# ocrickard/piper-swift

Hardware: AMD Instinct MI355X
Metric: audio-sec/wall-sec (RTF^-1) with ms/utterance, Piper VITS en_GB-medium geometry, scale-bench factor (higher is better)
Workload: dtype f32; 1 GPU; medium factor=8: 112 ids, 336 frames, 86016 samples (3.901 s audio) per utterance, 1 utterance per step per GPU; factor=8, phoneme_count=112, frames=336, samples=86016, parallelism=utterance-replicas x1 (one-shot RCCL weight broadcast)

## Files before the change

include/piper_hip.h:

```cpp
#ifndef PIPER_HIP_H
#define PIPER_HIP_H

#include <stddef.h>
#include <stdint.h>

#ifdef __cplusplus
extern "C" {
#endif

#define PIPER_HIP_ABI_VERSION 3

enum {
  PIPER_HIP_OK = 0,
  PIPER_HIP_ERR_SHAPE = -1,
  PIPER_HIP_ERR_TYPE = -2,
  PIPER_HIP_ERR_UNSUPPORTED = -3,
  PIPER_HIP_ERR_UNAVAILABLE = -4,
  PIPER_HIP_ERR_ALLOC = -5,
  PIPER_HIP_ERR_LAUNCH = -6,
  PIPER_HIP_ERR_ARG = -7
};

typedef struct piper_hip_ctx piper_hip_ctx;
typedef struct piper_hip_voice piper_hip_voice;
// ... 89 lines not shown
                               const int64_t* pads, float value, float** out, int64_t* out_shape,
                               piper_hip_stream stream);
int piper_hip_slice_f32(piper_hip_ctx* ctx, const float* x, const int64_t* shape, int rank, int axis, int64_t start,
                        int64_t end, int64_t step, float** out, int64_t* out_shape, piper_hip_stream stream);
int piper_hip_transpose_f32(piper_hip_ctx* ctx, const float* x, const int64_t* shape, int rank, const int32_t* perm,
                            float** out, int64_t* out_shape, piper_hip_stream stream);
int piper_hip_concat2_axis1_f32(piper_hip_ctx* ctx, const float* a, const int64_t a_shape[3], const float* b,
                                const int64_t b_shape[3], float** out, int64_t out_shape[3],
                                piper_hip_stream stream);
int piper_hip_split2_axis1_f32(piper_hip_ctx* ctx, const float* x, const int64_t x_shape[3], int64_t c0,
                               float** out0, float** out1, piper_hip_stream stream);
int piper_hip_expand_f32(piper_hip_ctx* ctx, const float* x, const int64_t* in_shape, const int64_t* out_shape,
                         int rank, float** out, piper_hip_stream stream);
int piper_hip_reduce_mean_lastdim_f32(piper_hip_ctx* ctx, const float* x, const int64_t* shape, int rank,
                                      float** out, piper_hip_stream stream);

int piper_hip_random_normal_like_f32(piper_hip_ctx* ctx, size_t count, uint64_t seed, float** out, piper_hip_stream stream);
int piper_hip_random_draws_u32(piper_hip_ctx* ctx, size_t count, uint64_t seed, uint32_t** out, piper_hip_stream stream);


int piper_hip_rel_attention_f32(piper_hip_ctx* ctx, const float* q, const float* k, const float* v,
                                const float* emb_rel_k, const float* emb_rel_v, int64_t n, int64_t heads,
                                int64_t head_dim, int64_t t, int64_t window, float** out, piper_hip_stream stream);

int piper_hip_attention_block_f32(piper_hip_ctx* ctx, const float* q, const float* k, const float* v, const float* emb_rel_k,
                                  const float* emb_rel_v, const float* w_o, const float* b_o, const float* x, const float* gamma,
                                  const float* beta, int64_t n, int64_t heads, int64_t head_dim, int64_t t, int64_t window, float eps,
                                  float** out, piper_hip_stream stream);

int piper_hip_add_layernorm_f32(piper_hip_ctx* ctx, const float* x, const float* y, const float* gamma,
                                const float* beta, int64_t n, int64_t c, int64_t t, float eps, float** out,
                                piper_hip_stream stream);

int piper_hip_wavenet_layer_f32(piper_hip_ctx* ctx, const float* x, const float* skip_in, const float* w_in,
                                const float* b_in, const float* w_rs, const float* b_rs, int64_t n, int64_t c,
                                int64_t t, int64_t k, int64_t dilation, int last, float** x_out, float** skip_out,
                                piper_hip_stream stream);

int piper_hip_hifigan_resblock_f32(piper_hip_ctx* ctx, int type, const float* x, int64_t n, int64_t c, int64_t t,
                                   int64_t k, const int32_t* dilations, int n_dil, const float* const* weights,
                                   const float* const* biases, float lrelu_slope, float** out,
                                   piper_hip_stream stream);


#define PIPER_HIP_MAX_UPS 4
#define PIPER_HIP_MAX_RB 3
// ... 266 lines not shown
```

piper-swift_amd/csrc/attention.hip:

```cpp
#include <algorithm>
#include <cstdlib>

#include "common.h"
#include "conv.h"

namespace {

constexpr int kBlock = 256;
constexpr int kKeyTile = 128;

__device__ __forceinline__ float wave_sum(float v) {
#pragma unroll
  for (int o = 32; o > 0; o >>= 1) v += __shfl_xor(v, o, 64);
  return v;
}
__device__ __forceinline__ float wave_max(float v) {
#pragma unroll
  for (int o = 32; o > 0; o >>= 1) v = fmaxf(v, __shfl_xor(v, o, 64));
  return v;
}

template <int R>
__global__ __launch_bounds__(kBlock) void rel_attention_kernel(const float* __restrict__ q, const float* __restrict__ k,
                                                               const float* __restrict__ v, const float* __restrict__ ek,
// ... 471 lines not shown
                    int T, int w, int64_t in_bs, int64_t out_bs, const int* len_ptr) {
  const int Tp = ((T + 31) / 32) * 32 + 2;
  const size_t lds = ((size_t)RV * Tp + 16 * 17) * sizeof(float);
  if (lds > 160 * 1024) return -1;
  static bool raised[ph::kMaxDevices] = {};
  if (lds > 64 * 1024 && ph::lds_optin_needed(raised))
    (void)hipFuncSetAttribute((const void*)rel_attention_mfma_kernel<D, RV>, hipFuncAttributeMaxDynamicSharedMemorySize, 160 * 1024);
  dim3 grid((unsigned)ph::ceil_div(T, RV), (unsigned)H, (unsigned)N);
  hipLaunchKernelGGL((rel_attention_mfma_kernel<D, RV>), grid, dim3(64 * kAttWaves), lds, s, q, k, v, ek, ev, out, T, w, in_bs, out_bs, len_ptr, Tp);
  return 0;
}

constexpr int kTK = 128;
constexpr int kLdK = kTK + 16;
constexpr int kLdV = kTK + 2;

#ifdef PH_ATT_LDS_TRACE
__device__ unsigned long long* ph_att_trace_buf;
#define PH_ASTAMP(k) do { if ((threadIdx.x & 63) == 0 && ph_att_trace_buf) ph_att_trace_buf[((size_t)(blockIdx.x + gridDim.x * blockIdx.y) * kAttWaves + (threadIdx.x >> 6)) * 8 + (k)] = __builtin_amdgcn_s_memtime(); } while (0)
#else
#define PH_ASTAMP(k) do { } while (0)
#endif
template <int D, bool SPLIT>
__global__ __launch_bounds__(64 * kAttWaves) void rel_attention_lds_kernel(const float* __restrict__ q, const float* __restrict__ k,
                                                                          const float* __restrict__ v, const float* __restrict__ ek,
                                                                          const float* __restrict__ ev, float* __restrict__ out, int T,
                                                                          int w, int64_t in_batch_stride, int64_t out_batch_stride,
                                                                          const int* __restrict__ len_ptr, int Tp, int nsplit,
                                                                          float* __restrict__ part_o, float* __restrict__ part_ml) {
  constexpr int RV = 16, NS = D / 4, NCT = D / 16;
  constexpr int NT = 64 * kAttWaves;
  constexpr int F4 = D * (kTK / 4);
  constexpr int SLOTS = (F4 + NT - 1) / NT;
  extern __shared__ __attribute__((aligned(16))) float smem[];
  float* tile = smem;
  float* sc = tile + D * kLdK;
  float* qs = sc + RV * Tp;
  float* qe = qs + D * 16;
  const int tid = threadIdx.x, lane = tid & 63;
  const int wave = __builtin_amdgcn_readfirstlane(tid >> 6);
  const int r16 = lane & 15, kq = lane >> 4;
  const int i0 = blockIdx.x * RV, n = blockIdx.z;
  const int h = SPLIT ? (int)blockIdx.y / nsplit : (int)blockIdx.y;
  const int part = SPLIT ? (int)blockIdx.y - h * nsplit : 0;
  const int Tv = len_ptr ? min(len_ptr[n], T) : T;
  if (i0 >= Tv) return;
  const int W = 2 * w + 1;
  const int64_t hoff = (int64_t)n * in_batch_stride + (int64_t)h * D * T;
  const float* qb = q + hoff;
  const float* kb = k + hoff;
  const float* vb = v + hoff;
  const float scale = sqrtf((float)D);
  const int ntile_all = (Tv + kTK - 1) / kTK;
  const int tpp = SPLIT ? (ntile_all + nsplit - 1) / nsplit : ntile_all;
  const int tb = SPLIT ? part * tpp : 0;
  const int te = SPLIT ? min(tb + tpp, ntile_all) : ntile_all;
  if (SPLIT && tb >= te) return;
  const int kbeg = tb * kTK, kend = min(te * kTK, Tv);
  const int ntile = te - tb;

  float4 stg[SLOTS];
  auto fetch = [&](const float* src, int t0) {
#pragma unroll
    for (int i = 0; i < SLOTS; i++) {
      const int e = tid + NT * i;
      const int row = min(e >> 5, D - 1), c4 = e & 31;
      const int col = min(t0 + 4 * c4, T - 4);
      stg[i] = *(const float4*)(src + (int64_t)row * T + col);
    }
  };
  auto commit = [&](int ld, int t0) {
#pragma unroll
    for (int i = 0; i < SLOTS; i++) {
      const int e = tid + NT * i;
      const int row = e >> 5, c4 = e & 31;
      if (row < D) {
        float4 val = stg[i];
        if (t0 + 4 * c4 > T - 4) val = make_float4(0.0f, 0.0f, 0.0f, 0.0f);
        float2* dst = (float2*)(tile + row * ld + 4 * c4);
        dst[0] = make_float2(val.x, val.y);
        dst[1] = make_float2(val.z, val.w);
      }
    }
  };

  PH_ASTAMP(0);
  fetch(kb, kbeg);
  for (int e = tid; e < D * 16; e += NT) {
    const int c = e >> 4, i = e & 15;
    const bool ok = i0 + i < Tv;
    const float qv = qb[(int64_t)c * T + min(i0 + i, Tv - 1)];
    qs[c * 16 + i] = ok ? qv / scale : 0.0f;
  }
  float arel[4];
  if (wave < NCT) {
#pragma unroll
    for (int s = 0; s < 4; s++) arel[s] = ev[min(4 * s + kq, W - 1) * D + wave * 16 + r16];
  }
  float ekf[NS];
  if (wave == kAttWaves - 1) {
    const int mc = min(r16, W - 1);
#pragma unroll
    for (int s = 0; s < NS; s++) ekf[s] = ek[mc * D + 4 * s + kq];
  }
  commit(kLdK, kbeg);
  PH_ASTAMP(1);
  __syncthreads();
  PH_ASTAMP(2);
  if (wave == kAttWaves - 1) {
    f32x4 a0 = {0.0f, 0.0f, 0.0f, 0.0f}, a1 = {0.0f, 0.0f, 0.0f, 0.0f};
#pragma unroll
    for (int s = 0; s < NS; s += 2) {
      a0 = __builtin_amdgcn_mfma_f32_16x16x4f32(qs[(4 * s + kq) * 16 + r16], r16 < W ? ekf[s] : 0.0f, a0, 0, 0, 0);
      a1 = __builtin_amdgcn_mfma_f32_16x16x4f32(qs[(4 * (s + 1) + kq) * 16 + r16], r16 < W ? ekf[s + 1] : 0.0f, a1, 0, 0, 0);
    }
#pragma unroll
    for (int r = 0; r < 4; r++) qe[(4 * kq + r) * 17 + r16] = a0[r] + a1[r];
  }

  for (int t = 0; t < ntile; t++) {
    const int t0 = kbeg + t * kTK;
    if (t + 1 < ntile) fetch(kb, t0 + kTK);
    else fetch(vb, kbeg);
    const int j0 = t0 + wave * 16;
    if (j0 < Tv) {
      const bool col_ok = j0 + r16 < Tv;
      f32x4 a0 = {0.0f, 0.0f, 0.0f, 0.0f}, a1 = {0.0f, 0.0f, 0.0f, 0.0f};
#pragma unroll
// ... 57 lines not shown
      row[j] = e;
      sum += e;
    }
    sum = wave_sum(sum);
    if constexpr (SPLIT) {
      if (lane == 0) {
        float* ml = part_ml + (((int64_t)n * gridDim.y + blockIdx.y) * 2) * T;
        ml[ia] = m;
        ml[T + ia] = sum;
      }
    } else {
      const float inv = 1.0f / sum;
      for (int j = lane; j < Tv; j += 64) row[j] *= inv;
    }
  }
  PH_ASTAMP(4);
  commit(kLdV, kbeg);
  __syncthreads();
  PH_ASTAMP(5);

  const bool pi_ok = i0 + r16 < Tv;
  const float* prow = sc + r16 * Tp;
  f32x4 acc = {0.0f, 0.0f, 0.0f, 0.0f}, accb = {0.0f, 0.0f, 0.0f, 0.0f};
  for (int t = 0; t < ntile; t++) {
    const int t0 = kbeg + t * kTK;
    if (t + 1 < ntile) fetch(vb, t0 + kTK);
    if (wave < NCT) {
      const float* vrow = tile + (wave * 16 + r16) * kLdV;
      const int nst = min(kTK, Tv - t0 + 3) >> 2;
      for (int s = 0; s < nst; s += 2) {
        const int j = t0 + 4 * s + kq;
        const bool ok = j < Tv, ok2 = j + 4 < Tv && s + 1 < nst;
        const float a0v = vrow[4 * s + kq], a1v = vrow[min(4 * (s + 1) + kq, kTK - 1)];
        const float b0v = prow[min(j, Tv - 1)], b1v = prow[min(j + 4, Tv - 1)];
        acc = __builtin_amdgcn_mfma_f32_16x16x4f32(ok ? a0v : 0.0f, (ok && pi_ok) ? b0v : 0.0f, acc, 0, 0, 0);
        accb = __builtin_amdgcn_mfma_f32_16x16x4f32(ok2 ? a1v : 0.0f, (ok2 && pi_ok) ? b1v : 0.0f, accb, 0, 0, 0);
      }
    }
    if (t + 1 < ntile) {
      __syncthreads();
      commit(kLdV, t0 + kTK);
      __syncthreads();
    }
  }
  if (wave < NCT) {
    const int ia = i0 + r16;
// ... 201 lines not shown
  const int Tp = ((T + 31) / 32) * 32 + 2;
  return ((size_t)2 * 16 * Tp + 2 * 16 * 17 + (size_t)H * d * 16 + kAttWaves * 16) * sizeof(float) <= 160 * 1024;
}

int launch_attention_block(piper_hip_ctx* ctx, hipStream_t s, const float* q, const float* k, const float* v, const float* ek, const float* ev,
                           const float* wo16, const float* bo, const float* xres, const float* gamma, const float* beta, float* out, int N,
                           int H, int d, int T, int w, int64_t in_batch_stride, int64_t x_batch_stride, const int* len_ptr, int o_nsteps,
                           float eps) {
  if (N <= 0 || T <= 0) return PIPER_HIP_OK;
  if (!attention_block_eligible(H, d, w, T) || N > 65535) PH_FAIL(PIPER_HIP_ERR_UNSUPPORTED, "attention_block: geometry not covered");
  if (launch_att_block<96>(s, q, k, v, ek, ev, wo16, bo, xres, gamma, beta, out, N, H, T, w, in_batch_stride, x_batch_stride, len_ptr, o_nsteps,
                           eps) != 0)
    PH_FAIL(PIPER_HIP_ERR_UNSUPPORTED, "attention_block: needs more than 160 KiB of LDS");
  PH_ROUTE(ctx, H * d, d, T, N, "att_block D=%d", d);
  hipError_t e = hipGetLastError();
  if (e != hipSuccess) PH_FAIL(PIPER_HIP_ERR_LAUNCH, "attention_block launch failed: %s", hipGetErrorString(e));
  return PIPER_HIP_OK;
}
}

PH_EXPORT int piper_hip_rel_attention_f32(piper_hip_ctx* ctx, const float* q, const float* k, const float* v,
                                          const float* emb_rel_k, const float* emb_rel_v, int64_t n, int64_t heads,
                                          int64_t head_dim, int64_t t, int64_t window, float** out, piper_hip_stream stream) {
  PH_CHECK_CTX(ctx);
  if (n < 0 || heads <= 0 || head_dim <= 0 || t < 0 || window < 0) PH_FAIL(PIPER_HIP_ERR_SHAPE, "rel_attention: bad shape");
  if (n * heads * head_dim * t > 0x7fffffff) PH_FAIL(PIPER_HIP_ERR_SHAPE, "rel_attention: tensor too large");
  const size_t cnt = (size_t)(n * heads * head_dim * t);
  int rc = ph::ensure_out(ctx, out, cnt, 0);
  if (rc) return rc;
  if (cnt == 0) return PIPER_HIP_OK;
  if (!q || !k || !v || !emb_rel_k || !emb_rel_v) PH_FAIL(PIPER_HIP_ERR_ARG, "rel_attention: null input");
  ph::StreamScope ss(ctx, stream);
  ph::RouteScope routes(ctx);
  const int64_t bs = heads * head_dim * t;
  const int nsplit = ph::rel_attention_split_parts(ctx, (int)n, (int)heads, (int)head_dim, (int)t, (int)window);
  if (nsplit > 1) {
    void *po = nullptr, *pml = nullptr;
    rc = ctx->pool.alloc((size_t)(n * heads * nsplit * head_dim * t) * sizeof(float), &po);
    if (rc) return rc;
    ph::defer_free(ctx, po);
    rc = ctx->pool.alloc((size_t)(n * heads * nsplit * 2 * t) * sizeof(float), &pml);
    if (rc) return rc;
    ph::defer_free(ctx, pml);
    rc = ph::launch_rel_attention_split(ctx, ss.s, q, k, v, emb_rel_k, emb_rel_v, *out, (int)n, (int)heads, (int)head_dim, (int)t, (int)window, bs,
                                        bs, nullptr, nsplit, (float*)po, (float*)pml);
  } else
    rc = ph::launch_rel_attention(ctx, ss.s, q, k, v, emb_rel_k, emb_rel_v, *out, (int)n, (int)heads, (int)head_dim, (int)t,
                                  (int)window, bs, bs, nullptr);
  if (rc) return rc;
  return ss.finish("rel_attention_f32");
}

PH_EXPORT int piper_hip_attention_block_f32(piper_hip_ctx* ctx, const float* q, const float* k, const float* v, const float* emb_rel_k,
                                            const float* emb_rel_v, const float* w_o, const float* b_o, const float* x,
                                            const float* gamma, const float* beta, int64_t n, int64_t heads, int64_t head_dim, int64_t t,
                                            int64_t window, float eps, float** out, piper_hip_stream stream) {
  PH_CHECK_CTX(ctx);
  if (n < 0 || heads <= 0 || head_dim <= 0 || t < 0 || window < 0) PH_FAIL(PIPER_HIP_ERR_SHAPE, "attention_block: bad shape");
  if (n * heads * head_dim * t > 0x7fffffff) PH_FAIL(PIPER_HIP_ERR_SHAPE, "attention_block: tensor too large");
  const int C = (int)(heads * head_dim);
  const size_t cnt = (size_t)(n * C * t);
  int rc = ph::ensure_out(ctx, out, cnt, 0);
  if (rc) return rc;
  if (cnt == 0) return PIPER_HIP_OK;
  if (!q || !k || !v || !emb_rel_k || !emb_rel_v || !w_o || !b_o || !x || !gamma || !beta) PH_FAIL(PIPER_HIP_ERR_ARG, "attention_block: null input");
  if (!ph::attention_block_eligible((int)heads, (int)head_dim, (int)window, (int)t))
    PH_FAIL(PIPER_HIP_ERR_UNSUPPORTED, "attention_block: covered geometry is head_dim 96, heads·head_dim ≤ 256, window ≤ 7, T ≤ 2048 — compose "
                                       "rel_attention + conv1d + add_layernorm instead");
  ph::StreamScope ss(ctx, stream);
  ph::RouteScope routes(ctx);
  void* pw = nullptr;
// ... 16 lines not shown
```

piper-swift_amd/csrc/prosody.hip:

```cpp
#include <algorithm>
#include <climits>
#include <cmath>

#include "common.h"
#include "dp_scalars.h"
#include "rng.h"

namespace ph {
namespace {

__global__ __launch_bounds__(256) void dp_final_prosody_kernel(const float* __restrict__ z, const float* __restrict__ m, const float* __restrict__ logs,
                                                               const DpScalars* __restrict__ sc, const float* __restrict__ len,
                                                               const int32_t* __restrict__ minf, const int32_t* __restrict__ maxf,
                                                               float* __restrict__ logw, float* __restrict__ w0_out, int32_t* __restrict__ dur, int T,
                                                               const int* __restrict__ len_ptr) {
  const int n = blockIdx.y;
  const int t = blockIdx.x * 256 + threadIdx.x;
  if (t >= T) return;
  const int64_t i = (int64_t)n * T + t;
  const float zv = z[(int64_t)n * 2 * T + t];
  const float lm = len[i];
  const int32_t mn = minf[i], mx = maxf[i];
  const float m0 = m[0], lg0 = logs[0], ls = sc[n].length_scale;
  const int Tv = len_ptr ? min(len_ptr[n], T) : T;
  float lw = 0.0f, w0 = 0.0f;
  int32_t d = 0;
  if (t < Tv) {
    lw = (zv - m0) * expf(-lg0);
// ... 74 lines not shown
    int32_t* tail = rep + n + (size_t)n * T;
    tail[b] = fitted ? 1 : 0;
    tail[n + 2 * b] = (int32_t)(unsigned)(S & 0xffffffffLL);
    tail[n + 2 * b + 1] = (int32_t)(S >> 32);
  }
  for (int f = tid; f < F; f += 256) {
    int id = 0;
    if (f < Fv && (long long)f < total) {
      int lo = 0, hi = Tb - 1;
      while (lo < hi) {
        const int mid = (lo + hi) >> 1;
        if (cum[mid] > f) hi = mid; else lo = mid + 1;
      }
      id = lo;
    }
    frame2id[(size_t)b * F + f] = id;
  }
}

__global__ __launch_bounds__(256) void expand_noise_prosody_kernel(const float* __restrict__ stats, const int32_t* __restrict__ frame2id,
                                                                   const float* __restrict__ noise, const float* __restrict__ id_noise,
                                                                   float* __restrict__ zp, float* __restrict__ zp_tap, int I, int T, int F,
                                                                   const float* __restrict__ noise_scale_dev, const unsigned* __restrict__ rng_dev,
                                                                   const int* __restrict__ lensF) {
  const int nb = blockIdx.y;
  stats += (int64_t)nb * 2 * I * T;
  frame2id += (int64_t)nb * F;
  noise += (int64_t)nb * I * F;
  id_noise += (int64_t)nb * T;
  zp += (int64_t)nb * I * F;
  zp_tap += (int64_t)nb * I * F;
  const float noise_scale = noise_scale_dev[nb];
  const bool gen = rng_dev[2 * nb] != 0u;
  const unsigned seed = rng_dev[2 * nb + 1];
  const int Fv = lensF ? min(lensF[nb], F) : F;
  const int64_t total = (int64_t)I * F;
  for (int64_t i = (int64_t)blockIdx.x * 256 + threadIdx.x; i < total; i += (int64_t)gridDim.x * 256) {
    const int c = (int)(i / F), f = (int)(i - (int64_t)c * F);
    const int t = frame2id[f];
    const float m = stats[(int64_t)c * T + t];
    const float lg = stats[(int64_t)(I + c) * T + t];
    const float pn = id_noise[t];
    const float nin = gen ? 0.0f : noise[i];
    const float nz = gen ? (f < Fv ? rnl_normal(seed, (unsigned)(c * Fv + f)) : 0.0f) : nin;
    const float ns = noise_scale * pn;
    const float r = m + (nz * expf(lg)) * ns;
    zp[i] = r;
    zp_tap[i] = r;
  }
}

const char* check_fields(const piper_hip_prosody* p, char* msg, size_t cap) {
  if (p->t < 1) { snprintf(msg, cap, "t = %d (at least 1)", p->t); return msg; }
  for (int i = 0; i < p->t; i++) {
    if (p->length && !(std::isfinite(p->length[i]) && p->length[i] >= 0.0f && p->length[i] <= 1000.0f)) {
      snprintf(msg, cap, "length[%d] = %g outside [0, 1000]", i, (double)p->length[i]);
      return msg;
    }
    if (p->noise && !(std::isfinite(p->noise[i]) && p->noise[i] >= 0.0f && p->noise[i] <= 1000.0f)) {
      snprintf(msg, cap, "noise[%d] = %g outside [0, 1000]", i, (double)p->noise[i]);
      return msg;
    }
    if (p->min_frames && (p->min_frames[i] < 0 || p->min_frames[i] > 1000000)) {
      snprintf(msg, cap, "min_frames[%d] = %d outside [0, 1000000]", i, p->min_frames[i]);
      return msg;
    }
    if (p->max_frames && (p->max_frames[i] < 0 || p->max_frames[i] > 1000000)) {
      snprintf(msg, cap, "max_frames[%d] = %d outside [0, 1000000]", i, p->max_frames[i]);
      return msg;
    }
    if (p->max_frames && p->min_frames && p->max_frames[i] != 0 && p->min_frames[i] > p->max_frames[i]) {
      snprintf(msg, cap, "min_frames[%d] = %d above max_frames[%d] = %d", i, p->min_frames[i], i, p->max_frames[i]);
// ... 13 lines not shown
    PH_FAIL(PIPER_HIP_ERR_ARG, "prosody: %s", why);
  }
  return PIPER_HIP_OK;
}

int launch_dp_final_prosody(hipStream_t s, const float* z, const float* m, const float* logs, const void* scalars, const float* len, const int32_t* minf,
                            const int32_t* maxf, float* logw, float* w0, int32_t* dur, int N, int T, const int* len_ptr) {
  const dim3 grid((unsigned)ceil_div(T, 256), (unsigned)N);
  hipLaunchKernelGGL(dp_final_prosody_kernel, grid, dim3(256), 0, s, z, m, logs, (const DpScalars*)scalars, len, minf, maxf, logw, w0, dur, T, len_ptr);
  return PIPER_HIP_OK;
}

size_t prosody_report_entries(int n, int T) { return (size_t)n + (size_t)n * T + 3 * (size_t)n; }

int launch_dp_paths_prosody(hipStream_t s, const int32_t* dur, const int* lensT, const int32_t* fit, int T, int F, int cap, int32_t* frame2id, int* lensF,
                            int32_t* rep, int n) {
  if (T > 4096 || !rep) PH_FAIL(PIPER_HIP_ERR_LAUNCH, "dp_paths_prosody: %d ids per row (at most 4096) or no report area", T);
  hipLaunchKernelGGL(dp_paths_prosody_kernel, dim3(n), dim3(256), 0, s, dur, lensT, fit, T, F, cap, frame2id, lensF, rep, n);
  return PIPER_HIP_OK;
}

int launch_expand_noise_prosody(hipStream_t s, const float* stats, const int32_t* frame2id, const float* noise, const float* id_noise, float* zp,
                                float* zp_tap, int NB, int I, int T, int F, const float* noise_scale, const unsigned* rng, const int* lensF) {
  const int grid = (int)std::min<int64_t>(ceil_div((int64_t)I * F, 256), 4096);
  hipLaunchKernelGGL(expand_noise_prosody_kernel, dim3(grid, NB), dim3(256), 0, s, stats, frame2id, noise, id_noise, zp, zp_tap, I, T, F, noise_scale, rng,
                     lensF);
  return PIPER_HIP_OK;
}

}
namespace ph { namespace { PH_WARM(prosody, dp_final_prosody_kernel); } }

using namespace ph;

PH_EXPORT int piper_hip_prosody_check(const piper_hip_prosody* p) { return prosody_check_item(p, -1); }

PH_EXPORT int piper_hip_prosody_frames(const piper_hip_prosody* p, const float* w0, int32_t t, int64_t cap, int32_t* frames_out, int64_t* wanted) {
  if (!w0 || !frames_out) PH_FAIL(PIPER_HIP_ERR_ARG, "prosody_frames: null argument");
  if (t < 1) PH_FAIL(PIPER_HIP_ERR_ARG, "prosody_frames: t = %d (at least 1)", t);
  if (p) {
    if (int rc = prosody_check_item(p, -1)) return rc;
    if (p->t != t) PH_FAIL(PIPER_HIP_ERR_SHAPE, "prosody_frames: the prosody has %d entries, the utterance %d ids", p->t, t);
  }
  int64_t S = 0;
  for (int i = 0; i < t; i++) {
    const float w1 = w0[i] * ((p && p->length) ? p->length[i] : 1.0f);
    const float c = ceilf(w1);
    const int32_t d0 = c > 0.0f ? (c < 1e6f ? (int32_t)c : 1000000) : 0;
    const int32_t mx = (p && p->max_frames) ? p->max_frames[i] : 0, mn = (p && p->min_frames) ? p->min_frames[i] : 0;
// ... 10 lines not shown
```

piper-swift_amd/csrc/voice.hip:

```cpp
#include <algorithm>
#include <cmath>
#include <cstdlib>
#include <chrono>
#include <functional>
#include <memory>

#include "../../include/piper_hip_voice_layout.h"
#include "conv.h"
#include "conv_bf16.h"
#include "conv_win.h"
#include "pcm16.h"
#include "resample.h"
#include "rng.h"
#include "speaker.h"

namespace ph {
int validate_config(const piper_hip_voice_config* c);
int validate_speaker_config(const piper_hip_voice_config* cfg, const piper_hip_speaker_config* sc);
int launch_rel_attention(piper_hip_ctx* ctx, hipStream_t s, const float* q, const float* k, const float* v, const float* ek,
                         const float* ev, float* out, int N, int H, int d, int T, int w, int64_t in_batch_stride,
                         int64_t out_batch_stride, const int* len_ptr);
int rel_attention_split_parts(piper_hip_ctx* ctx, int N, int H, int d, int T, int w);
int launch_rel_attention_split(piper_hip_ctx* ctx, hipStream_t s, const float* q, const float* k, const float* v, const float* ek,
                               const float* ev, float* out, int N, int H, int d, int T, int w, int64_t in_batch_stride,
                               int64_t out_batch_stride, const int* len_ptr, int nsplit, float* part_o, float* part_ml);
size_t dp_scalars_bytes(int n);
void dp_scalars_fill(void* host, int i, float noise_w, float length_scale, unsigned gen, unsigned seed);
bool flow_seam_eligible(int H, int half);
int launch_flow_seam(piper_hip_ctx* ctx, hipStream_t s, const float* skip, float* zp, float* h, const float* post16, const float* post_b, const float* pre16,
                     const float* pre_b, int N, int H, int half, int F, int post_steps, int pre_steps, int ob, int os, const int* len_ptr);
bool dds_layer_eligible(int H, int K);
int launch_dds_layer(piper_hip_ctx* ctx, hipStream_t s, const float* x, const float* dw_w, const float* dw_b, const float* g1, const float* b1,
                     const float* pw16, const float* pw_b, const float* g2, const float* b2, float* out, int N, int H, int T, int K, int dil,
// ... 21 lines not shown
using namespace ph;

namespace {

constexpr int kBlock = 256;
constexpr int kMaxSlots = 16;

__global__ __launch_bounds__(kBlock) void embed_kernel(const int64_t* __restrict__ ids, const float* __restrict__ emb,
                                                       float* __restrict__ x, int H, int T, int n_vocab, float scale) {
  ids += (int64_t)blockIdx.y * T;
  x += (int64_t)blockIdx.y * H * T;
  const int total = H * T;
  for (int i = blockIdx.x * kBlock + threadIdx.x; i < total; i += gridDim.x * kBlock) {
    const int c = i / T, t = i - c * T;
    int64_t id = ids[t];
    if (id < 0) id += n_vocab;
    x[i] = (id < 0 || id >= n_vocab) ? 0.0f * scale : emb[id * H + c] * scale;
  }
}

__global__ __launch_bounds__(kBlock) void expand_noise_kernel(const float* __restrict__ stats, const int32_t* __restrict__ frame2id,
                                                              const float* __restrict__ noise, float* __restrict__ zp, float* __restrict__ zp_tap,
                                                              int I, int T, int F, const float* __restrict__ noise_scale_dev,
                                                              const unsigned* __restrict__ rng_dev, const int* __restrict__ lensF) {
  const int nb = blockIdx.y;
  stats += (int64_t)nb * 2 * I * T;
  frame2id += (int64_t)nb * F;
  noise += (int64_t)nb * I * F;
  zp += (int64_t)nb * I * F;
  zp_tap += (int64_t)nb * I * F;
  const float noise_scale = noise_scale_dev[nb];
  const bool gen = rng_dev[2 * nb] != 0u;
  const unsigned seed = rng_dev[2 * nb + 1];
  const int Fv = lensF ? min(lensF[nb], F) : F;
  const int64_t total = (int64_t)I * F;
  for (int64_t i = (int64_t)blockIdx.x * kBlock + threadIdx.x; i < total; i += (int64_t)gridDim.x * kBlock) {
    const int c = (int)(i / F), f = (int)(i - (int64_t)c * F);
    const int t = frame2id[f];
    const float m = stats[(int64_t)c * T + t];
    const float lg = stats[(int64_t)(I + c) * T + t];
    const float nz = gen ? (f < Fv ? rnl_normal(seed, (unsigned)(c * Fv + f)) : 0.0f) : noise[i];
    const float r = m + (nz * expf(lg)) * noise_scale;
    zp[i] = r;
    zp_tap[i] = r;
  }
}

__global__ __launch_bounds__(kBlock) void mrf_mean_lrelu_kernel(const float* __restrict__ a, const float* __restrict__ b,
                                                                const float* __restrict__ c, float* __restrict__ y, int64_t n,
                                                                float alpha) {
  const int64_t n4 = n >> 2;
  const int64_t stride = (int64_t)gridDim.x * kBlock;
  for (int64_t i = (int64_t)blockIdx.x * kBlock + threadIdx.x; i < n4; i += stride) {
    const float4 va = reinterpret_cast<const float4*>(a)[i], vb = reinterpret_cast<const float4*>(b)[i],
                 vc = reinterpret_cast<const float4*>(c)[i];
    float4 r;
    r.x = ((va.x + vb.x) + vc.x) / 3.0f; r.y = ((va.y + vb.y) + vc.y) / 3.0f;
    r.z = ((va.z + vb.z) + vc.z) / 3.0f; r.w = ((va.w + vb.w) + vc.w) / 3.0f;
    r.x = r.x >= 0.0f ? r.x : alpha * r.x; r.y = r.y >= 0.0f ? r.y : alpha * r.y;
    r.z = r.z >= 0.0f ? r.z : alpha * r.z; r.w = r.w >= 0.0f ? r.w : alpha * r.w;
    reinterpret_cast<float4*>(y)[i] = r;
  }
  for (int64_t i = (n4 << 2) + (int64_t)blockIdx.x * kBlock + threadIdx.x; i < n; i += stride) {
    const float v = ((a[i] + b[i]) + c[i]) / 3.0f;
    y[i] = v >= 0.0f ? v : alpha * v;
  }
}

// ... 1381 lines not shown
    b.conv("enc.proj", v->proj, b.plain(x, stats, H, 2 * I, T, lensT), T);
  return PIPER_HIP_OK;
}

const float* build_flow(Builder& b, const FrontBuffers& fb) {
  piper_hip_voice* v = b.v;
  Slot& s = b.s;
  const int T = b.T, F = b.F, NB = b.NB;
  const int* lensF = b.lensF;
  const piper_hip_voice_config& c = v->cfg;
  const int H = c.hidden, I = c.inter;
  float *stats = fb.stats, *zp = fb.zp, *zflip = fb.zflip, *zp_tap = fb.zp_tap, *h = fb.h, *acts = fb.acts, *skip = fb.skip;
  {
    const int32_t* f2i = s.frame2id;
    const float* nz = s.noise;
    const float* nsd = s.noise_scale;
    const unsigned* rngd = s.rng;
    if (s.pro) {
      const float* idn = s.pro_noise;
      b.step("expand_noise_prosody", "", NB * 2.0 * 2.0 * F * (double)I * T, NB * 2.0 * 4.0 * ((double)F * T + (double)T * I + (double)F * I),
             [=](hipStream_t q) { return launch_expand_noise_prosody(q, stats, f2i, nz, idn, zp, zp_tap, NB, I, T, F, nsd, rngd, lensF); });
    } else
    b.step("expand_noise", "", NB * 2.0 * 2.0 * F * (double)I * T, NB * 2.0 * 4.0 * ((double)F * T + (double)T * I + (double)F * I), [=](hipStream_t q) {
      const int grid = (int)std::min<int64_t>(ceil_div((int64_t)I * F, kBlock), 4096);
      hipLaunchKernelGGL(expand_noise_kernel, dim3(grid, NB), dim3(kBlock), 0, q, stats, f2i, nz, zp, zp_tap, I, T, F, nsd, rngd, lensF);
      return PIPER_HIP_OK;
    });
  }
  b.tap("z_p", zp_tap, I, F, 1);
  bool flipped = false;
  const int half = I / 2;
  static const bool no_seam = getenv("PIPER_HIP_NO_FLOW_SEAM") != nullptr;
  auto seam_ok = [&](const piper_hip_voice::Coupling& A, const piper_hip_voice::Coupling& B) {
    return !no_seam && I == 2 * half && flow_seam_eligible(H, half) && A.post.w16 && B.pre.w16 && A.post.bias && B.pre.bias && A.post.K == 1 && B.pre.K == 1 &&
           A.post.Cin == H && A.post.Cout == half && B.pre.Cin == half && B.pre.Cout == H;
  };
  static const bool no_fold = getenv("PIPER_HIP_NO_FLOW_FOLD") != nullptr;
  bool fold = !no_fold && c.wn_layers >= 2 && flow_tail_plan_ok(v->ctx, H, half, F, NB);
  for (int f = 0; f < c.n_flows && fold; f++)
    fold = v->flows[f].tail_w && v->flows[f].tail_b && (f == 0 || seam_ok(v->flows[f], v->flows[f - 1]));
  float* zloc[2] = {zp, zp};
  for (int f = c.n_flows - 1; f >= 0; f--) {
    flipped = !flipped;
    const auto& C = v->flows[f];
    const std::string p = "flow" + std::to_string(f) + ".";
    const bool pre_done = f + 1 < c.n_flows && (fold || seam_ok(v->flows[f + 1], C));
    if (!pre_done) {
      ConvArgs a = b.plain(zp, h, I, H, F, lensF);
// ... 3205 lines not shown
```

piper-swift_amd/python/piper_hip/__init__.py:

```python
import ctypes as C
import os

import numpy as np

_HERE = os.path.dirname(os.path.abspath(__file__))
LIB_PATH = os.path.normpath(os.path.join(_HERE, "..", "..", "lib", "libpiper_hip.so"))
LIB_NORT_PATH = os.path.normpath(os.path.join(_HERE, "..", "..", "lib", "libpiper_hip_nort.so"))



class ExecutionError(RuntimeError):
    code = None


class ShapeMismatch(ExecutionError):
    code = -1


class TypeMismatch(ExecutionError):
    code = -2


class UnsupportedOp(ExecutionError):
    code = -3
# ... 213 lines not shown
                                                C.POINTER(ConvTranspose1dParams), C.POINTER(c_vp), c_i64p, c_vp]),
    "piper_hip_conv1d_bf16": (C.c_int, [c_vp, c_vp, c_i64p, c_vp, c_i64p, c_vp, C.POINTER(Conv1dParams),
                                        C.POINTER(c_vp), c_i64p, c_vp]),
    "piper_hip_convtranspose1d_bf16": (C.c_int, [c_vp, c_vp, c_i64p, c_vp, c_i64p, c_vp,
                                                 C.POINTER(ConvTranspose1dParams), C.POINTER(c_vp), c_i64p, c_vp]),
    "piper_hip_matmul_f32": (C.c_int, [c_vp, c_vp, c_i64p, c_vp, c_i64p, C.c_int, C.POINTER(c_vp), c_i64p, c_vp]),
    "piper_hip_softmax_lastdim_f32": (C.c_int, [c_vp, c_vp, c_i64p, C.c_int, C.POINTER(c_vp), c_vp]),
    "piper_hip_unary_f32": (C.c_int, [c_vp, C.c_int, c_vp, C.c_size_t, C.c_float, C.POINTER(c_vp), c_vp]),
    "piper_hip_binary_broadcast_f32": (C.c_int, [c_vp, C.c_int, c_vp, c_i64p, C.c_int, c_vp, c_i64p, C.c_int,
                                                 C.POINTER(c_vp), c_i64p, C.POINTER(C.c_int), c_vp]),
    "piper_hip_pad_constant_f32": (C.c_int, [c_vp, c_vp, c_i64p, C.c_int, c_i64p, C.c_float, C.POINTER(c_vp), c_i64p,
                                             c_vp]),
    "piper_hip_slice_f32": (C.c_int, [c_vp, c_vp, c_i64p, C.c_int, C.c_int, C.c_int64, C.c_int64, C.c_int64,
                                      C.POINTER(c_vp), c_i64p, c_vp]),
    "piper_hip_transpose_f32": (C.c_int, [c_vp, c_vp, c_i64p, C.c_int, c_i32p, C.POINTER(c_vp), c_i64p, c_vp]),
    "piper_hip_concat2_axis1_f32": (C.c_int, [c_vp, c_vp, c_i64p, c_vp, c_i64p, C.POINTER(c_vp), c_i64p, c_vp]),
    "piper_hip_split2_axis1_f32": (C.c_int, [c_vp, c_vp, c_i64p, C.c_int64, C.POINTER(c_vp), C.POINTER(c_vp), c_vp]),
    "piper_hip_expand_f32": (C.c_int, [c_vp, c_vp, c_i64p, c_i64p, C.c_int, C.POINTER(c_vp), c_vp]),
    "piper_hip_reduce_mean_lastdim_f32": (C.c_int, [c_vp, c_vp, c_i64p, C.c_int, C.POINTER(c_vp), c_vp]),
    "piper_hip_random_normal_like_f32": (C.c_int, [c_vp, C.c_size_t, C.c_uint64, C.POINTER(c_vp), c_vp]),
    "piper_hip_random_draws_u32": (C.c_int, [c_vp, C.c_size_t, C.c_uint64, C.POINTER(c_vp), c_vp]),
    "piper_hip_rel_attention_f32": (C.c_int, [c_vp, c_vp, c_vp, c_vp, c_vp, c_vp, C.c_int64, C.c_int64, C.c_int64,
                                              C.c_int64, C.c_int64, C.POINTER(c_vp), c_vp]),
    "piper_hip_attention_block_f32": (C.c_int, [c_vp] * 11 + [C.c_int64] * 5 + [C.c_float, C.POINTER(c_vp), c_vp]),
    "piper_hip_add_layernorm_f32": (C.c_int, [c_vp, c_vp, c_vp, c_vp, c_vp, C.c_int64, C.c_int64, C.c_int64, C.c_float,
                                              C.POINTER(c_vp), c_vp]),
    "piper_hip_wavenet_layer_f32": (C.c_int, [c_vp, c_vp, c_vp, c_vp, c_vp, c_vp, c_vp, C.c_int64, C.c_int64, C.c_int64,
                                              C.c_int64, C.c_int64, C.c_int, C.POINTER(c_vp), C.POINTER(c_vp), c_vp]),
    "piper_hip_hifigan_resblock_f32": (C.c_int, [c_vp, C.c_int, c_vp, C.c_int64, C.c_int64, C.c_int64, C.c_int64, c_i32p,
                                                 C.c_int, C.POINTER(c_vp), C.POINTER(c_vp), C.c_float, C.POINTER(c_vp),
                                                 c_vp]),
    "piper_hip_voice_config_preset": (C.c_int, [C.c_int, C.POINTER(VoiceConfig)]),
    "piper_hip_voice_blob_floats": (C.c_int, [C.POINTER(VoiceConfig), C.POINTER(C.c_size_t)]),
    "piper_hip_voice_blob_layout": (C.c_int, [C.POINTER(VoiceConfig), C.POINTER(TensorInfo), C.c_int,
                                              C.POINTER(C.c_int)]),
    "piper_hip_voice_synthetic_blob": (C.c_int, [C.POINTER(VoiceConfig), C.c_uint64, c_f32p, C.c_size_t]),
    "piper_hip_voice_create": (C.c_int, [c_vp, C.POINTER(VoiceConfig), c_vp, C.c_int, C.POINTER(c_vp)]),
    "piper_hip_onnx_open": (C.c_int, [C.c_char_p, C.POINTER(c_vp)]),
    "piper_hip_onnx_open_memory": (C.c_int, [c_vp, C.c_size_t, C.POINTER(c_vp)]),
    "piper_hip_onnx_close": (None, [c_vp]),
    "piper_hip_onnx_counts": (C.c_int, [c_vp, C.POINTER(C.c_int64), C.POINTER(C.c_int64), C.POINTER(C.c_int),
                                        C.POINTER(C.c_int)]),
    "piper_hip_onnx_initializer": (C.c_int, [c_vp, C.c_int, C.POINTER(OnnxTensorInfo)]),
    "piper_hip_onnx_find": (C.c_int, [c_vp, C.c_char_p]),
    "piper_hip_onnx_read_f32": (C.c_int, [c_vp, C.c_int, c_f32p, C.c_size_t]),
    "piper_hip_onnx_infer_config": (C.c_int, [c_vp, C.POINTER(VoiceConfig)]),
# ... 450 lines not shown
        return DeviceBuffer(self, p.value, got.value, owned=out is None, dtype=np.int16)

    def g711F32(self, buf, law, inRate=None, outRate=None, gain=1.0, count=None, out=None, commandBuffer=None):
        n = buf.count if count is None else int(count)
        p = c_vp(_ptr(out)) if out is not None else c_vp()
        got = C.c_size_t()
        r_in = 1 if inRate is None else int(inRate)
        r_out = r_in if outRate is None else int(outRate)
        _check(self.lib.piper_hip_g711_f32(self.ctx, _ptr(buf), n, r_in, r_out, float(gain), _law(law), C.byref(p), C.byref(got), commandBuffer))
        return DeviceBuffer(self, p.value, got.value, owned=out is None, dtype=np.uint8)

    def downloadUint8(self, buf, count=None):
        n = buf.count if count is None else int(count)
        out = np.empty((n + 3) // 4 * 4, np.uint8)
        _check(self.lib.piper_hip_download_f32(self.ctx, _ptr(buf), out.ctypes.data_as(c_f32p), (n + 3) // 4))
        return out[:n].copy()

    def downloadInt16(self, buf, count=None):
        n = buf.count if count is None else int(count)
        out = np.empty(n + 1, np.int16)
        _check(self.lib.piper_hip_download_f32(self.ctx, _ptr(buf), out.ctypes.data_as(c_f32p), (n + 1) // 2))
        return out[:n].copy()

    def relAttentionF32(self, q, k, v, embRelK, embRelV, n, heads, headDim, t, window, commandBuffer=None):
        p = c_vp()
        _check(self.lib.piper_hip_rel_attention_f32(self.ctx, _ptr(q), _ptr(k), _ptr(v), _ptr(embRelK), _ptr(embRelV), n,
                                                    heads, headDim, t, window, C.byref(p), commandBuffer))
        return self._out(p, [n, heads * headDim, t])

    def attentionBlockF32(self, q, k, v, embRelK, embRelV, wO, bO, x, gamma, beta, n, heads, headDim, t, window, eps=1e-5,
                          commandBuffer=None):
        p = c_vp()
        _check(self.lib.piper_hip_attention_block_f32(self.ctx, _ptr(q), _ptr(k), _ptr(v), _ptr(embRelK), _ptr(embRelV), _ptr(wO), _ptr(bO),
                                                      _ptr(x), _ptr(gamma), _ptr(beta), n, heads, headDim, t, window, eps, C.byref(p),
                                                      commandBuffer))
        return self._out(p, [n, heads * headDim, t])

    def addLayerNormF32(self, x, y, gamma, beta, n, c, t, eps=1e-5, commandBuffer=None):
        p = c_vp()
        _check(self.lib.piper_hip_add_layernorm_f32(self.ctx, _ptr(x), _ptr(y), _ptr(gamma), _ptr(beta), n, c, t, eps,
                                                    C.byref(p), commandBuffer))
        return self._out(p, [n, c, t])

    def wavenetLayerF32(self, x, skipIn, wIn, bIn, wRs, bRs, n, c, t, k, dilation, last, commandBuffer=None):
        px, ps = c_vp(), c_vp()
        _check(self.lib.piper_hip_wavenet_layer_f32(self.ctx, _ptr(x), _ptr(skipIn), _ptr(wIn), _ptr(bIn), _ptr(wRs),
                                                    _ptr(bRs), n, c, t, k, dilation, int(bool(last)), C.byref(px),
                                                    C.byref(ps), commandBuffer))
        xo = None if last else self._out(px, [n, c, t])[0]
        return xo, self._out(ps, [n, c, t])[0]
# ... 915 lines not shown
```

Baseline: 5804 audio-sec/wall-sec.

## Prefetch attention operands before length check, add single-tile PV path, vectorize noise expansion

The LDS attention kernel now issues its K tile, Q and relative-embedding loads before reading the per-batch length, so the length read no longer serializes global loads, and it raises occupancy through a launch_bounds minimum-blocks hint. It adds a specialised PV loop for the single-key-tile case. The expand_noise kernels are merged into a shared body with a float4-vectorised path that uses one block row per channel. A lens-aware rel_attention entry point is also exported. Risks include register pressure from the min-blocks hint and extra speculative loads for blocks that exit early.

```diff
diff --git a/include/piper_hip.h b/include/piper_hip.h
--- a/include/piper_hip.h
+++ b/include/piper_hip.h
@@ -135,6 +135,9 @@
 int piper_hip_rel_attention_f32(piper_hip_ctx* ctx, const float* q, const float* k, const float* v,
                                 const float* emb_rel_k, const float* emb_rel_v, int64_t n, int64_t heads,
                                 int64_t head_dim, int64_t t, int64_t window, float** out, piper_hip_stream stream);
+int piper_hip_rel_attention_lens_f32(piper_hip_ctx* ctx, const float* q, const float* k, const float* v,
+                                     const float* emb_rel_k, const float* emb_rel_v, const int32_t* lens, int64_t n, int64_t heads,
+                                     int64_t head_dim, int64_t t, int64_t window, float** out, piper_hip_stream stream);
 
 int piper_hip_attention_block_f32(piper_hip_ctx* ctx, const float* q, const float* k, const float* v, const float* emb_rel_k,
                                   const float* emb_rel_v, const float* w_o, const float* b_o, const float* x, const float* gamma,
diff --git a/piper-swift_amd/csrc/attention.hip b/piper-swift_amd/csrc/attention.hip
--- a/piper-swift_amd/csrc/attention.hip
+++ b/piper-swift_amd/csrc/attention.hip
@@ -517,7 +517,7 @@
 #define PH_ASTAMP(k) do { } while (0)
 #endif
 template <int D, bool SPLIT>
-__global__ __launch_bounds__(64 * kAttWaves) void rel_attention_lds_kernel(const float* __restrict__ q, const float* __restrict__ k,
+__global__ __launch_bounds__(64 * kAttWaves, 4) void rel_attention_lds_kernel(const float* __restrict__ q, const float* __restrict__ k,
                                                                           const float* __restrict__ v, const float* __restrict__ ek,
                                                                           const float* __restrict__ ev, float* __restrict__ out, int T,
                                                                           int w, int64_t in_batch_stride, int64_t out_batch_stride,
@@ -527,6 +527,7 @@
   constexpr int NT = 64 * kAttWaves;
   constexpr int F4 = D * (kTK / 4);
   constexpr int SLOTS = (F4 + NT - 1) / NT;
+  constexpr int QS = (D * 16 + NT - 1) / NT;
   extern __shared__ __attribute__((aligned(16))) float smem[];
   float* tile = smem;
   float* sc = tile + D * kLdK;
@@ -538,21 +539,12 @@
   const int i0 = blockIdx.x * RV, n = blockIdx.z;
   const int h = SPLIT ? (int)blockIdx.y / nsplit : (int)blockIdx.y;
   const int part = SPLIT ? (int)blockIdx.y - h * nsplit : 0;
-  const int Tv = len_ptr ? min(len_ptr[n], T) : T;
-  if (i0 >= Tv) return;
   const int W = 2 * w + 1;
   const int64_t hoff = (int64_t)n * in_batch_stride + (int64_t)h * D * T;
   const float* qb = q + hoff;
   const float* kb = k + hoff;
   const float* vb = v + hoff;
   const float scale = sqrtf((float)D);
-  const int ntile_all = (Tv + kTK - 1) / kTK;
-  const int tpp = SPLIT ? (ntile_all + nsplit - 1) / nsplit : ntile_all;
-  const int tb = SPLIT ? part * tpp : 0;
-  const int te = SPLIT ? min(tb + tpp, ntile_all) : ntile_all;
-  if (SPLIT && tb >= te) return;
-  const int kbeg = tb * kTK, kend = min(te * kTK, Tv);
-  const int ntile = te - tb;
 
   float4 stg[SLOTS];
   auto fetch = [&](const float* src, int t0) {
@@ -578,27 +570,56 @@
       }
     }
   };
-
+  float qv[QS];
+  auto fetch_q = [&](int last) {
+#pragma unroll
+    for (int i = 0; i < QS; i++) {
+      const int e = min(tid + NT * i, D * 16 - 1);
+      qv[i] = qb[(int64_t)(e >> 4) * T + min(i0 + (e & 15), last)];
+    }
+  };
+  float arel[4];
+  float ekf[NS];
+  auto fetch_rel = [&]() {
+    if (wave < NCT) {
+#pragma unroll
+      for (int s = 0; s < 4; s++) arel[s] = ev[min(4 * s + kq, W - 1) * D + wave * 16 + r16];
+    }
+    if (wave == kAttWaves - 1) {
+      const int mc = min(r16, W - 1);
+#pragma unroll
+      for (int s = 0; s < NS; s++) ekf[s] = ek[mc * D + 4 * s + kq];
+    }
+  };
   PH_ASTAMP(0);
-  fetch(kb, kbeg);
-  for (int e = tid; e < D * 16; e += NT) {
-    const int c = e >> 4, i = e & 15;
-    const bool ok = i0 + i < Tv;
-    const float qv = qb[(int64_t)c * T + min(i0 + i, Tv - 1)];
-    qs[c * 16 + i] = ok ? qv / scale : 0.0f;
-  }
-  float arel[4];
-  if (wave < NCT) {
-#pragma unroll
-    for (int s = 0; s < 4; s++) arel[s] = ev[min(4 * s + kq, W - 1) * D + wave * 16 + r16];
-  }
-  float ekf[NS];
-  if (wave == kAttWaves - 1) {
-    const int mc = min(r16, W - 1);
-#pragma unroll
-    for (int s = 0; s < NS; s++) ekf[s] = ek[mc * D + 4 * s + kq];
+  if constexpr (!SPLIT) {
+    fetch(kb, 0);
+    fetch_q(T - 1);
+    fetch_rel();
+    __builtin_amdgcn_sched_barrier(0);
+  }
+  const int Tv = len_ptr ? min(len_ptr[n], T) : T;
+  if (i0 >= Tv) return;
+  const int ntile_all = (Tv + kTK - 1) / kTK;
+  const int tpp = SPLIT ? (ntile_all + nsplit - 1) / nsplit : ntile_all;
+  const int tb = SPLIT ? part * tpp : 0;
+  const int te = SPLIT ? min(tb + tpp, ntile_all) : ntile_all;
+  if (SPLIT && tb >= te) return;
+  const int kbeg = tb * kTK, kend = min(te * kTK, Tv);
+  const int ntile = te - tb;
+
+  if constexpr (SPLIT) {
+    fetch(kb, kbeg);
+    fetch_q(Tv - 1);
+    fetch_rel();
+  }
+#pragma unroll
+  for (int i = 0; i < QS; i++) {
+    const int e = tid + NT * i;
+    if (e < D * 16) qs[e] = i0 + (e & 15) < Tv ? qv[i] / scale : 0.0f;
   }
   commit(kLdK, kbeg);
+  const bool one_tile = !SPLIT && ntile == 1;
   PH_ASTAMP(1);
   __syncthreads();
   PH_ASTAMP(2);
@@ -702,6 +723,32 @@
   const bool pi_ok = i0 + r16 < Tv;
   const float* prow = sc + r16 * Tp;
   f32x4 acc = {0.0f, 0.0f, 0.0f, 0.0f}, accb = {0.0f, 0.0f, 0.0f, 0.0f};
+  if (one_tile) {
+    if (wave < NCT) {
+      const float* vrow = tile + (wave * 16 + r16) * kLdV + kq;
+      const float* pr = prow + kq;
+#pragma unroll
+      for (int s0 = 0; s0 < kTK / 4; s0 += 8) {
+        float av[8], bv[8];
+#pragma unroll
+        for (int u = 0; u < 8; u++) {
+          av[u] = vrow[4 * (s0 + u)];
+          bv[u] = pr[4 * (s0 + u)];
+        }
+#pragma unroll
+        for (int u = 0; u < 8; u++) {
+          const bool ok = 4 * (s0 + u) + kq < Tv;
+          av[u] = ok ? av[u] : 0.0f;
+          bv[u] = (ok && pi_ok) ? bv[u] : 0.0f;
+        }
+#pragma unroll
+        for (int u = 0; u < 8; u += 2) {
+          acc = __builtin_amdgcn_mfma_f32_16x16x4f32(av[u], bv[u], acc, 0, 0, 0);
+          accb = __builtin_amdgcn_mfma_f32_16x16x4f32(av[u + 1], bv[u + 1], accb, 0, 0, 0);
+        }
+      }
+    }
+  } else
   for (int t = 0; t < ntile; t++) {
     const int t0 = kbeg + t * kTK;
     if (t + 1 < ntile) fetch(vb, t0 + kTK);
@@ -949,6 +996,13 @@
 PH_EXPORT int piper_hip_rel_attention_f32(piper_hip_ctx* ctx, const float* q, const float* k, const float* v,
                                           const float* emb_rel_k, const float* emb_rel_v, int64_t n, int64_t heads,
                                           int64_t head_dim, int64_t t, int64_t window, float** out, piper_hip_stream stream) {
+  return piper_hip_rel_attention_lens_f32(ctx, q, k, v, emb_rel_k, emb_rel_v, nullptr, n, heads, head_dim, t, window, out, stream);
+}
+
+PH_EXPORT int piper_hip_rel_attention_lens_f32(piper_hip_ctx* ctx, const float* q, const float* k, const float* v,
+                                               const float* emb_rel_k, const float* emb_rel_v, const int32_t* lens, int64_t n,
+                                               int64_t heads, int64_t head_dim, int64_t t, int64_t window, float** out,
+                                               piper_hip_stream stream) {
   PH_CHECK_CTX(ctx);
   if (n < 0 || heads <= 0 || head_dim <= 0 || t < 0 || window < 0) PH_FAIL(PIPER_HIP_ERR_SHAPE, "rel_attention: bad shape");
   if (n * heads * head_dim * t > 0x7fffffff) PH_FAIL(PIPER_HIP_ERR_SHAPE, "rel_attention: tensor too large");
@@ -970,10 +1024,10 @@
     if (rc) return rc;
     ph::defer_free(ctx, pml);
     rc = ph::launch_rel_attention_split(ctx, ss.s, q, k, v, emb_rel_k, emb_rel_v, *out, (int)n, (int)heads, (int)head_dim, (int)t, (int)window, bs,
-                                        bs, nullptr, nsplit, (float*)po, (float*)pml);
+                                        bs, lens, nsplit, (float*)po, (float*)pml);
   } else
     rc = ph::launch_rel_attention(ctx, ss.s, q, k, v, emb_rel_k, emb_rel_v, *out, (int)n, (int)heads, (int)head_dim, (int)t,
-                                  (int)window, bs, bs, nullptr);
+                                  (int)window, bs, bs, lens);
   if (rc) return rc;
   return ss.finish("rel_attention_f32");
 }
diff --git a/piper-swift_amd/csrc/expand_noise.h b/piper-swift_amd/csrc/expand_noise.h
--- /dev/null
+++ b/piper-swift_amd/csrc/expand_noise.h
@@ -0,0 +1,90 @@
+#pragma once
+#include <hip/hip_runtime.h>
+
+#include <cstdint>
+
+#include "rng.h"
+
+namespace ph {
+
+inline bool expand_noise_vec_ok(const int32_t* frame2id, const float* noise, const float* zp, const float* zp_tap, const int* lensF, int NB, int I,
+                                int F) {
+  return noise && lensF && F >= 4 && (F & 3) == 0 && I >= 1 && I <= 65535 && NB >= 1 && NB <= 65535 &&
+         (((uintptr_t)frame2id | (uintptr_t)noise | (uintptr_t)zp | (uintptr_t)zp_tap) & 15) == 0;
+}
+inline dim3 expand_noise_grid(bool vec, int NB, int I, int F) {
+  if (vec) return dim3((unsigned)((F / 4 + 255) / 256), (unsigned)I, (unsigned)NB);
+  const int64_t blocks = ((int64_t)I * F + 255) / 256;
+  return dim3((unsigned)(blocks < 4096 ? blocks : 4096), (unsigned)NB);
+}
+
+template <bool PROSODY>
+__device__ __forceinline__ void expand_noise_body(const float* __restrict__ stats, const int32_t* __restrict__ frame2id, const float* __restrict__ noise,
+                                                  const float* __restrict__ id_noise, float* __restrict__ zp, float* __restrict__ zp_tap, int I, int T,
+                                                  int F, const float* __restrict__ noise_scale_dev, const unsigned* __restrict__ rng_dev,
+                                                  const int* __restrict__ lensF, int vec) {
+  if (vec) {
+    const int nb = blockIdx.z, c = blockIdx.y;
+    const int f = 4 * (int)(blockIdx.x * 256 + threadIdx.x);
+    if (f >= F) return;
+    const float* st = stats + (int64_t)nb * 2 * I * T;
+    const int64_t row = ((int64_t)nb * I + c) * F + f;
+    const int4 t4 = *(const int4*)(frame2id + (int64_t)nb * F + f);
+    const float4 n4 = *(const float4*)(noise + row);
+    __builtin_amdgcn_sched_barrier(0);
+    const float noise_scale = noise_scale_dev[nb];
+    const unsigned gen_u = rng_dev[2 * nb], seed = rng_dev[2 * nb + 1];
+    const int lf = lensF[nb];
+    __builtin_amdgcn_sched_barrier(0);
+    const int tt[4] = {t4.x, t4.y, t4.z, t4.w};
+    const float nin[4] = {n4.x, n4.y, n4.z, n4.w};
+    float m[4], lg[4], pn[4];
+#pragma unroll
+    for (int k = 0; k < 4; k++) {
+      m[k] = st[(int64_t)c * T + tt[k]];
+      lg[k] = st[(int64_t)(I + c) * T + tt[k]];
+      pn[k] = PROSODY ? id_noise[(int64_t)nb * T + tt[k]] : 0.0f;
+    }
+    __builtin_amdgcn_sched_barrier(0);
+    const bool gen = gen_u != 0u;
+    const int Fv = min(lf, F);
+    float r[4];
+#pragma unroll
+    for (int k = 0; k < 4; k++) {
+      const float nz = gen ? (f + k < Fv ? rnl_normal(seed, (unsigned)(c * Fv + f + k)) : 0.0f) : nin[k];
+      const float ns = PROSODY ? noise_scale * pn[k] : noise_scale;
+      r[k] = m[k] + (nz * expf(lg[k])) * ns;
+    }
+    const float4 r4 = make_float4(r[0], r[1], r[2], r[3]);
+    *(float4*)(zp + row) = r4;
+    *(float4*)(zp_tap + row) = r4;
+    return;
+  }
+  const int nb = blockIdx.y;
+  stats += (int64_t)nb * 2 * I * T;
+  frame2id += (int64_t)nb * F;
+  noise += (int64_t)nb * I * F;
+  if (PROSODY) id_noise += (int64_t)nb * T;
+  zp += (int64_t)nb * I * F;
+  zp_tap += (int64_t)nb * I * F;
+  const float noise_scale = noise_scale_dev[nb];
+  const bool gen = rng_dev[2 * nb] != 0u;
+  const unsigned seed = rng_dev[2 * nb + 1];
+  const int Fv = lensF ? min(lensF[nb], F) : F;
+  const int64_t total = (int64_t)I * F;
+  for (int64_t i = (int64_t)blockIdx.x * 256 + threadIdx.x; i < total; i += (int64_t)gridDim.x * 256) {
+    const int c = (int)(i / F), f = (int)(i - (int64_t)c * F);
+    const int t = frame2id[f];
+    const float m = stats[(int64_t)c * T + t];
+    const float lg = stats[(int64_t)(I + c) * T + t];
+    const float pn = PROSODY ? id_noise[t] : 0.0f;
+    const float nin = gen ? 0.0f : noise[i];
+    const float nz = gen ? (f < Fv ? rnl_normal(seed, (unsigned)(c * Fv + f)) : 0.0f) : nin;
+    const float ns = PROSODY ? noise_scale * pn : noise_scale;
+    const float r = m + (nz * expf(lg)) * ns;
+    zp[i] = r;
+    zp_tap[i] = r;
+  }
+}
+
+}
diff --git a/piper-swift_amd/csrc/prosody.hip b/piper-swift_amd/csrc/prosody.hip
--- a/piper-swift_amd/csrc/prosody.hip
+++ b/piper-swift_amd/csrc/prosody.hip
@@ -4,6 +4,7 @@
 
 #include "common.h"
 #include "dp_scalars.h"
+#include "expand_noise.h"
 #include "rng.h"
 
 namespace ph {
@@ -124,32 +125,8 @@
                                                                    const float* __restrict__ noise, const float* __restrict__ id_noise,
                                                                    float* __restrict__ zp, float* __restrict__ zp_tap, int I, int T, int F,
                                                                    const float* __restrict__ noise_scale_dev, const unsigned* __restrict__ rng_dev,
-                                                                   const int* __restrict__ lensF) {
-  const int nb = blockIdx.y;
-  stats += (int64_t)nb * 2 * I * T;
-  frame2id += (int64_t)nb * F;
-  noise += (int64_t)nb * I * F;
-  id_noise += (int64_t)nb * T;
-  zp += (int64_t)nb * I * F;
-  zp_tap += (int64_t)nb * I * F;
-  const float noise_scale = noise_scale_dev[nb];
-  const bool gen = rng_dev[2 * nb] != 0u;
-  const unsigned seed = rng_dev[2 * nb + 1];
-  const int Fv = lensF ? min(lensF[nb], F) : F;
-  const int64_t total = (int64_t)I * F;
-  for (int64_t i = (int64_t)blockIdx.x * 256 + threadIdx.x; i < total; i += (int64_t)gridDim.x * 256) {
-    const int c = (int)(i / F), f = (int)(i - (int64_t)c * F);
-    const int t = frame2id[f];
-    const float m = stats[(int64_t)c * T + t];
-    const float lg = stats[(int64_t)(I + c) * T + t];
-    const float pn = id_noise[t];
-    const float nin = gen ? 0.0f : noise[i];
-    const float nz = gen ? (f < Fv ? rnl_normal(seed, (unsigned)(c * Fv + f)) : 0.0f) : nin;
-    const float ns = noise_scale * pn;
-    const float r = m + (nz * expf(lg)) * ns;
-    zp[i] = r;
-    zp_tap[i] = r;
-  }
+                                                                   const int* __restrict__ lensF, int vec) {
+  expand_noise_body<true>(stats, frame2id, noise, id_noise, zp, zp_tap, I, T, F, noise_scale_dev, rng_dev, lensF, vec);
 }
 
 const char* check_fields(const piper_hip_prosody* p, char* msg, size_t cap) {
@@ -209,9 +186,9 @@
 
 int launch_expand_noise_prosody(hipStream_t s, const float* stats, const int32_t* frame2id, const float* noise, const float* id_noise, float* zp,
                                 float* zp_tap, int NB, int I, int T, int F, const float* noise_scale, const unsigned* rng, const int* lensF) {
-  const int grid = (int)std::min<int64_t>(ceil_div((int64_t)I * F, 256), 4096);
-  hipLaunchKernelGGL(expand_noise_prosody_kernel, dim3(grid, NB), dim3(256), 0, s, stats, frame2id, noise, id_noise, zp, zp_tap, I, T, F, noise_scale, rng,
-                     lensF);
+  const bool vec = expand_noise_vec_ok(frame2id, noise, zp, zp_tap, lensF, NB, I, F) && ((uintptr_t)id_noise & 3) == 0;
+  hipLaunchKernelGGL(expand_noise_prosody_kernel, expand_noise_grid(vec, NB, I, F), dim3(256), 0, s, stats, frame2id, noise, id_noise, zp, zp_tap, I, T, F,
+                     noise_scale, rng, lensF, vec ? 1 : 0);
   return PIPER_HIP_OK;
 }
 
diff --git a/piper-swift_amd/csrc/voice.hip b/piper-swift_amd/csrc/voice.hip
--- a/piper-swift_amd/csrc/voice.hip
+++ b/piper-swift_amd/csrc/voice.hip
@@ -9,6 +9,7 @@
 #include "conv.h"
 #include "conv_bf16.h"
 #include "conv_win.h"
+#include "expand_noise.h"
 #include "pcm16.h"
 #include "resample.h"
 #include "rng.h"
@@ -76,28 +77,8 @@
 __global__ __launch_bounds__(kBlock) void expand_noise_kernel(const float* __restrict__ stats, const int32_t* __restrict__ frame2id,
                                                               const float* __restrict__ noise, float* __restrict__ zp, float* __restrict__ zp_tap,
                                                               int I, int T, int F, const float* __restrict__ noise_scale_dev,
-                                                              const unsigned* __restrict__ rng_dev, const int* __restrict__ lensF) {
-  const int nb = blockIdx.y;
-  stats += (int64_t)nb * 2 * I * T;
-  frame2id += (int64_t)nb * F;
-  noise += (int64_t)nb * I * F;
-  zp += (int64_t)nb * I * F;
-  zp_tap += (int64_t)nb * I * F;
-  const float noise_scale = noise_scale_dev[nb];
-  const bool gen = rng_dev[2 * nb] != 0u;
-  const unsigned seed = rng_dev[2 * nb + 1];
-  const int Fv = lensF ? min(lensF[nb], F) : F;
-  const int64_t total = (int64_t)I * F;
-  for (int64_t i = (int64_t)blockIdx.x * kBlock + threadIdx.x; i < total; i += (int64_t)gridDim.x * kBlock) {
-    const int c = (int)(i / F), f = (int)(i - (int64_t)c * F);
-    const int t = frame2id[f];
-    const float m = stats[(int64_t)c * T + t];
-    const float lg = stats[(int64_t)(I + c) * T + t];
-    const float nz = gen ? (f < Fv ? rnl_normal(seed, (unsigned)(c * Fv + f)) : 0.0f) : noise[i];
-    const float r = m + (nz * expf(lg)) * noise_scale;
-    zp[i] = r;
-    zp_tap[i] = r;
-  }
+                                                              const unsigned* __restrict__ rng_dev, const int* __restrict__ lensF, int vec) {
+  expand_noise_body<false>(stats, frame2id, noise, nullptr, zp, zp_tap, I, T, F, noise_scale_dev, rng_dev, lensF, vec);
 }
 
 __global__ __launch_bounds__(kBlock) void mrf_mean_lrelu_kernel(const float* __restrict__ a, const float* __restrict__ b,
@@ -1525,8 +1506,9 @@
              [=](hipStream_t q) { return launch_expand_noise_prosody(q, stats, f2i, nz, idn, zp, zp_tap, NB, I, T, F, nsd, rngd, lensF); });
     } else
     b.step("expand_noise", "", NB * 2.0 * 2.0 * F * (double)I * T, NB * 2.0 * 4.0 * ((double)F * T + (double)T * I + (double)F * I), [=](hipStream_t q) {
-      const int grid = (int)std::min<int64_t>(ceil_div((int64_t)I * F, kBlock), 4096);
-      hipLaunchKernelGGL(expand_noise_kernel, dim3(grid, NB), dim3(kBlock), 0, q, stats, f2i, nz, zp, zp_tap, I, T, F, nsd, rngd, lensF);
+      const bool vec = expand_noise_vec_ok(f2i, nz, zp, zp_tap, lensF, NB, I, F);
+      hipLaunchKernelGGL(expand_noise_kernel, expand_noise_grid(vec, NB, I, F), dim3(kBlock), 0, q, stats, f2i, nz, zp, zp_tap, I, T, F, nsd, rngd, lensF,
+                         vec ? 1 : 0);
       return PIPER_HIP_OK;
     });
   }
diff --git a/piper-swift_amd/python/piper_hip/__init__.py b/piper-swift_amd/python/piper_hip/__init__.py
--- a/piper-swift_amd/python/piper_hip/__init__.py
+++ b/piper-swift_amd/python/piper_hip/__init__.py
@@ -259,6 +259,8 @@
     "piper_hip_random_draws_u32": (C.c_int, [c_vp, C.c_size_t, C.c_uint64, C.POINTER(c_vp), c_vp]),
     "piper_hip_rel_attention_f32": (C.c_int, [c_vp, c_vp, c_vp, c_vp, c_vp, c_vp, C.c_int64, C.c_int64, C.c_int64,
                                               C.c_int64, C.c_int64, C.POINTER(c_vp), c_vp]),
+    "piper_hip_rel_attention_lens_f32": (C.c_int, [c_vp, c_vp, c_vp, c_vp, c_vp, c_vp, c_vp, C.c_int64, C.c_int64, C.c_int64,
+                                                   C.c_int64, C.c_int64, C.POINTER(c_vp), c_vp]),
     "piper_hip_attention_block_f32": (C.c_int, [c_vp] * 11 + [C.c_int64] * 5 + [C.c_float, C.POINTER(c_vp), c_vp]),
     "piper_hip_add_layernorm_f32": (C.c_int, [c_vp, c_vp, c_vp, c_vp, c_vp, C.c_int64, C.c_int64, C.c_int64, C.c_float,
                                               C.POINTER(c_vp), c_vp]),
@@ -755,10 +757,14 @@
         _check(self.lib.piper_hip_download_f32(self.ctx, _ptr(buf), out.ctypes.data_as(c_f32p), (n + 1) // 2))
         return out[:n].copy()
 
-    def relAttentionF32(self, q, k, v, embRelK, embRelV, n, heads, headDim, t, window, commandBuffer=None):
+    def relAttentionF32(self, q, k, v, embRelK, embRelV, n, heads, headDim, t, window, commandBuffer=None, lens=None):
         p = c_vp()
-        _check(self.lib.piper_hip_rel_attention_f32(self.ctx, _ptr(q), _ptr(k), _ptr(v), _ptr(embRelK), _ptr(embRelV), n,
-                                                    heads, headDim, t, window, C.byref(p), commandBuffer))
+        if lens is None:
+            _check(self.lib.piper_hip_rel_attention_f32(self.ctx, _ptr(q), _ptr(k), _ptr(v), _ptr(embRelK), _ptr(embRelV), n,
+                                                        heads, headDim, t, window, C.byref(p), commandBuffer))
+        else:
+            _check(self.lib.piper_hip_rel_attention_lens_f32(self.ctx, _ptr(q), _ptr(k), _ptr(v), _ptr(embRelK), _ptr(embRelV), _ptr(lens), n,
+                                                             heads, headDim, t, window, C.byref(p), commandBuffer))
         return self._out(p, [n, heads * headDim, t])
 
     def attentionBlockF32(self, q, k, v, embRelK, embRelV, wO, bO, x, gamma, beta, n, heads, headDim, t, window, eps=1e-5,
```

Result: no change. 5861 audio-sec/wall-sec (median of 6 runs) (+1.0%).
